# mozack/vdjer

Measured on NVIDIA B200. Metric: graph_build_prune_windows_per_sec, higher is better.
Workload: dtype u8/u64

## Files before the change

vdjer_b200/csrc/kernels.cuh:

```cuda
#pragma once
#include <cstdint>
#include <cuda_runtime.h>

namespace vdjg {

typedef unsigned long long u64;
typedef unsigned int u32;
typedef unsigned short u16;
typedef unsigned char u8;

constexpr u64 EMPTY64 = ~0ull;
constexpr u64 INF64 = ~0ull;
constexpr u32 NIL32 = 0xFFFFFFFFu;
constexpr u32 CNT_CAP = 32765;
constexpr int GATE_Q = 20;
constexpr int HIQ = 30;
constexpr int FLB = 6;
constexpr u32 CNT2_MASK = 0x00FFFFFFu;
constexpr int CNT2_IN = 24;
constexpr u64 LOG_A = 1ull << 62, LOG_B = 1ull << 63;
constexpr int QSUM_SAT = 214;
constexpr int MAX_LOG_RANKS = 11;
constexpr u32 CNT_MULTI = 0x80000000u;
constexpr u32 CNT_SURV = 0x40000000u;
constexpr u32 CNT_MASK = 0x3FFFFFFFu;
constexpr int THREADS = 256;
constexpr int WARPS = THREADS / 32;
constexpr u32 LOG_CHUNK = 64;
constexpr u32 MAX_PROBE = 1u << 14;
constexpr int HIST_BITS = 8;
constexpr int NBUCKET = 1 << HIST_BITS;
constexpr int BHLL_BITS = 7;
constexpr int BHLL = 1 << BHLL_BITS;
constexpr int BATCH = 4;
#ifndef PASS1_MIN_BLOCKS
#define PASS1_MIN_BLOCKS 4
#endif
#ifndef PASS2_MIN_BLOCKS
#define PASS2_MIN_BLOCKS 3
#endif
constexpr int MINI_M = 10;
constexpr int RUN_MAX = 24;
constexpr int SEG_MAX = 32;
constexpr int STAMP_BITS = 40;

struct __align__(32) Slot1 {
    u64 klo, khi;
    u32 count;
    u32 head;
    u32 first_rec;
    u32 first_fp;
};
static_assert(sizeof(Slot1) == 32, "Slot1 must be one sector");

struct __align__(64) Slot2 {
    u64 klo, khi;
    u32 count;
    u32 rank;
    u64 first_any;
    u64 out_first[4];
};
static_assert(sizeof(Slot2) == 64, "Slot2 must be two sectors");


struct Geom {
    int L, k, w, nb, nm;
    int seg;
    int segs;
    u32 tile_rec;
    u64 R;
    u64 n_tiles;
    u64 kmask_lo, kmask_hi;
// ... 176 lines not shown

__device__ __forceinline__ void kmer_succ(u64 lo, u64 hi, u32 c, int k, u64 &slo, u64 &shi) {
    slo = (lo >> 2) | (hi << 62);
    shi = hi >> 2;
    int bit = 2 * (k - 1);
    if (bit < 64) slo |= (u64)c << bit; else shi |= (u64)c << (bit - 64);
}
__device__ __forceinline__ void kmer_pred(u64 lo, u64 hi, u32 c, u64 mlo, u64 mhi, u64 &plo, u64 &phi) {
    phi = ((hi << 2) | (lo >> 62)) & mhi;
    plo = ((lo << 2) | (u64)c) & mlo;
}
__device__ __forceinline__ u32 kmer_last(u64 lo, u64 hi, int k) {
    int bit = 2 * (k - 1);
    return (u32)(bit < 64 ? lo >> bit : hi >> (bit - 64)) & 3u;
}

__device__ __forceinline__ u32 kmer_bucket_of(u64 lo, u64 hi, int span, u32 mmask) {
    u32 minh = ~0u;
    for (int j = 0; j < span; j++) {
        minh = min(minh, mini_hash((u32)lo & mmask));
        lo = (lo >> 2) | (hi << 62);
        hi >>= 2;
    }
    return mini_bucket(minh);
}

template <bool WIDE>
__device__ __forceinline__ void tuple_decode(const Part &pt, u64 w1, u64 w2, u64 &hi, u32 &fl, u32 &fp, u64 &stamp) {
    hi = pt.hb ? (w1 & ((1ull << pt.hb) - 1)) : 0ull;
    fl = (u32)(w1 >> pt.hb) & ((1u << FLB) - 1);
    fp = (u32)(w1 >> (pt.hb + FLB)) & (u32)((1ull << pt.fb) - 1);
    stamp = WIDE ? w2 : (w1 >> (pt.hb + FLB + pt.fb));
}
__device__ __forceinline__ void issue_fence(u32 &a, u32 &b, u32 &c, u32 &d) {
    asm volatile("" : "+r"(a), "+r"(b), "+r"(c), "+r"(d));
}

struct PackArgs {
    const unsigned char *text;
    u64 r0, n;
    u32 fwd_only;
    u64 *bases, *good, *valid, *hiq;
    u8 *qual, *strand;
    u64 *bad;
};
__device__ __forceinline__ u64 spread_bits(u32 a) {
    u64 x = a;
    x = (x | (x << 16)) & 0x0000FFFF0000FFFFull;
    x = (x | (x << 8)) & 0x00FF00FF00FF00FFull;
    x = (x | (x << 4)) & 0x0F0F0F0F0F0F0F0Full;
    x = (x | (x << 2)) & 0x3333333333333333ull;
    x = (x | (x << 1)) & 0x5555555555555555ull;
    return x;
}
__device__ __forceinline__ void pack_record(const PackArgs &a, const Geom &g, const unsigned char *rec, u64 r, bool rev, u32 lane) {
    if (lane == 0) {
        const unsigned sc = rec[0];
        if (sc != '0' && sc != '1') atomicMin(&a.bad[0], r);
        if (sc == '1') a.bad[2] = 1;
        a.strand[r] = (u8)(sc - '0');
    }
    u64 vword = 0, gword = 0, hword = 0;
    for (int j0 = 0; j0 < g.L; j0 += 32) {
        const int j = j0 + (int)lane;
        unsigned code = 4;
        bool okq = false, hiq = false;
        if (j < g.L) {
            const int sj = rev ? g.L - 1 - j : j;
// ... 508 lines not shown
    __device__ __forceinline__ void setup(unsigned char *smem) {
        unsigned char *p = smem + (threadIdx.x >> 5) * bytes();
        lo = reinterpret_cast<u64 *>(p);
        w1 = lo + QC;
        w2 = w1 + QC;
        idx = reinterpret_cast<u32 *>(w1 + (WIDE ? 2 : 1) * QC);
    }
    __host__ __device__ static constexpr size_t bytes() { return (size_t)QC * (WIDE ? 28 : 20); }
    template <class Make>
    __device__ __forceinline__ u32 push_lazy(u32 qn, bool defer, u64 l, u32 i, Make make) {
        const u32 lane = threadIdx.x & 31;
        const u32 ballot = __ballot_sync(0xFFFFFFFFu, defer);
        if (defer) {
            const u32 pos = qn + __popc(ballot & ((1u << lane) - 1));
            u64 a, b;
            make(a, b);
            lo[pos] = l; w1[pos] = a; idx[pos] = i;
            if (WIDE) w2[pos] = b;
        }
        return qn + __popc(ballot);
    }
    __device__ __forceinline__ u32 push(u32 qn, bool defer, u64 l, u64 a, u64 b, u32 i) {
        const u32 lane = threadIdx.x & 31;
        const u32 ballot = __ballot_sync(0xFFFFFFFFu, defer);
        if (defer) {
            const u32 pos = qn + __popc(ballot & ((1u << lane) - 1));
            lo[pos] = l; w1[pos] = a; idx[pos] = i;
            if (WIDE) w2[pos] = b;
        }
        return qn + __popc(ballot);
    }
};

struct RunCursor {
    u64 w0, w1, w2;
    u64 stamp0;
    u32 off, len;
    u32 l;
    u32 j;
    u32 rem;
};
struct RunFeed {
    u64 *rw;
    u32 cnt, incl, total;
    u32 live;
    template <bool GATED_ONLY>
    __device__ __forceinline__ static u32 selected(u64 w2) {
        return GATED_ONLY ? (u32)w2 & 0xFFFFFFu : (1u << run_len(w2)) - 1u;
    }
    template <bool GATED_ONLY>
    __device__ __forceinline__ void load(const u64 *runs, u64 ri, u64 n_runs) {
        const u32 lane = threadIdx.x & 31;
        u64 w0 = 0, w1 = 0, w2 = 0, w3 = 0;
        cnt = 0;
        if (ri < n_runs) {
            ld_run(runs + ri * RUN_WORDS, w0, w1, w2, w3);
            cnt = (u32)__popc(selected<GATED_ONLY>(w2));
        }
        incl = cnt;
        for (int o = 1; o < 32; o <<= 1) { const u32 v = __shfl_up_sync(0xFFFFFFFFu, incl, o); if ((int)lane >= o) incl += v; }
        total = __shfl_sync(0xFFFFFFFFu, incl, 31);
        live = __ballot_sync(0xFFFFFFFFu, cnt != 0);
        __syncwarp();
        u64 *p = rw + lane * RUN_WORDS;
        p[0] = w0; p[1] = w1; p[2] = ri < n_runs ? w2 : 0ull; p[3] = w3;
        __syncwarp();
    }
    template <bool TAB2>
    __device__ __forceinline__ void open(RunCursor &c, const Part &pt) const {
        const u64 *p = rw + c.l * RUN_WORDS;
        c.w0 = p[0]; c.w1 = p[1]; c.w2 = p[2];
        const u64 w3 = p[3];
        c.stamp0 = w3 & ((1ull << STAMP_BITS) - 1);
        const uint4 ut = __ldg(reinterpret_cast<const uint4 *>(pt.ut + (run_bucket(w3) >> pt.ushift)));
        c.off = TAB2 ? ut.z : ut.x;
        c.len = TAB2 ? ut.w : ut.y;
    }
    template <bool GATED_ONLY, bool TAB2>
    __device__ __forceinline__ void seek(u32 t, RunCursor &c, const Part &pt) const {
        u32 l = 0;
#pragma unroll
        for (int s = 16; s; s >>= 1) { const u32 v = __shfl_sync(0xFFFFFFFFu, incl, l + s - 1); if (v <= t) l += s; }
        u32 nth = t - __shfl_sync(0xFFFFFFFFu, incl - cnt, l);
        c.l = l;
        open<TAB2>(c, pt);
        u32 m = selected<GATED_ONLY>(c.w2), j = 0;
        if (GATED_ONLY) {
#pragma unroll
            for (int s = 16; s; s >>= 1) {
                const u32 k = (u32)__popc(m & ((1u << s) - 1u));
                if (nth >= k) { nth -= k; m >>= s; j += s; }
            }
            m >>= 1;
        } else {
            j = nth;
            m >>= j + 1;
        }
        c.j = j; c.rem = m;
    }
    __device__ __forceinline__ u32 fingerprint(u32 l, const Part &pt) const {
        const u64 *p = rw + l * RUN_WORDS;
        return (((u32)(p[3] >> 48) & 0xFFFFu) | (((u32)(p[2] >> 58) & 0x3Fu) << 16)) & (u32)((1ull << pt.fb) - 1);
    }
    template <bool GATED_ONLY, bool TAB2>
    __device__ __forceinline__ void next(RunCursor &c, const Part &pt) const {
        if (c.rem) {
            const u32 s = (u32)__ffs((int)c.rem);
            c.j += s; c.rem >>= s;
            return;
        }
        const u32 ahead = c.l < 31 ? live >> (c.l + 1) : 0u;
        c.l += ahead ? (u32)__ffs((int)ahead) : 0u;
        open<TAB2>(c, pt);
        const u32 m = selected<GATED_ONLY>(c.w2);
        const u32 s = m ? (u32)__ffs((int)m) : 1u;
        c.j = s - 1; c.rem = m >> s;
    }
};
__device__ __forceinline__ void run_kmer(const Geom &g, const RunCursor &c, u64 &lo, u64 &hi, u32 &idx) {
    const u32 sh = 2u * c.j;
    lo = sh ? (c.w0 >> sh) | (c.w1 << (64 - sh)) : c.w0;
    hi = c.w1 >> sh;
    lo &= g.kmask_lo; hi &= g.kmask_hi;
    idx = slot_in(hash_slot(lo, hi), c.off, c.len);
}
__device__ __forceinline__ u32 run_flags(const Geom &g, u64 w0, u64 w1, u64 w2, u32 j) {
    const u32 p = j + (u32)g.k;
    const u32 nb = (u32)((p < 32 ? w0 >> (2 * p) : w1 >> (2 * (p - 32)))) & 3u;
    const bool has_next = j + 1 < run_len(w2) || ((w2 >> 53) & 1ull);
    return (has_next ? 1u | (nb << 1) : 0u) | ((u32)(w2 >> (24 + j)) & 1u) << 3 | ((u32)(w2 >> 54) & 1u) << 4;
}
__device__ __forceinline__ u32 run_flags2(const Geom &g, u64 w0, u64 w1, u64 w2, u32 j) {
    const u32 p = j + (u32)g.k;
    const u32 nb = (u32)((p < 32 ? w0 >> (2 * p) : w1 >> (2 * (p - 32)))) & 3u;
    const bool has_next = j + 1 < run_len(w2) || ((w2 >> 53) & 1ull);
    const u32 prev = j ? 1u | (((u32)(w0 >> (2 * (j - 1))) & 3u) << 1) : (u32)(w2 >> 55) & 7u;
    return (has_next ? 1u | (nb << 1) : 0u) | prev << 3;
}
template <bool WIDE>
__device__ __forceinline__ void pack_tuple(const Part &pt, u64 hi, u32 fl, u32 fp, u64 stamp, u64 &t1, u64 &t2) {
    t1 = hi | ((u64)fl << pt.hb) | ((u64)fp << (pt.hb + FLB));
    if (WIDE) t2 = stamp;
    else { t1 |= stamp << (pt.hb + FLB + pt.fb); t2 = 0; }
}

struct LogCursor { u32 base, used; };

template <bool WIDE>
__device__ __forceinline__ u32 pass1_drain(const Pass1Args &a, const Geom &g, const Part &pt, WarpQueue<WIDE, QCAP1> &q,
                                           u32 qn, LogCursor &lc, bool final) {
    const u32 lane = threadIdx.x & 31, lt = (1u << lane) - 1;
    u32 next = 0;
    bool have = false;
    u64 lo = 0, hi = 0, stamp = 0, rw1 = 0, rw2 = 0;
    u32 idx = 0, probe = 0, fp = 0, fl = 0;
    __syncwarp();
    for (;;) {
        const u32 need = __ballot_sync(0xFFFFFFFFu, !have);
        const u32 avail = qn - next;
        if (avail == 0 && (need == 0xFFFFFFFFu || (!final && 32 - __popc(need) < (int)pt.qdense1))) break;
        if (need && avail) {
            const u32 my = __popc(need & lt);
            if (!have && my < avail) {
                const u32 e = next + my;
                lo = q.lo[e]; rw1 = q.w1[e]; rw2 = WIDE ? q.w2[e] : 0ull;
                tuple_decode<WIDE>(pt, rw1, rw2, hi, fl, fp, stamp);
                idx = q.idx[e];
                probe = 0;
                have = true;
            }
// ... 43 lines not shown
                if (a.nb_ranks && blk != NIL32) a.log[(u64)blk * a.nb_ranks] = entry;
                st_cg_u64(reinterpret_cast<u64 *>(&slot->first_rec), (u64)r | ((u64)fp << 32));
            } else {
                const u32 cw = (u32)q2, cnt = cw & CNT_MASK;
                const u32 first_rec = (u32)q3, first_fp = (u32)(q3 >> 32);
                u32 rank = NIL32;
                if (cnt + 1 < a.nb_ranks) rank = (atomicAdd(&slot->count, 1u) & CNT_MASK) + 1;
                else if (cnt + 1 < CNT_CAP) atomicAdd(&slot->count, 1u);
                if (!(cw & CNT_MULTI) && first_rec != r &&
                    (first_fp != fp || !same_read(a.rd, first_rec, r, g.nb, g.nm)))
                    atomicOr(&slot->count, CNT_MULTI);
                if (rank < a.nb_ranks && blk != NIL32) a.log[(u64)blk * a.nb_ranks + rank] = entry;
            }
            have = false;
        }
    }
    __syncwarp();
    const u32 left = q.push(0, have, lo, rw1, rw2, idx);
    __syncwarp();
    return left;
}

__device__ __forceinline__ void hot_flush(Slot1 *table, u32 *hidx, u32 *hcnt) {
    for (u32 i = threadIdx.x & 31; i < HOTC; i += 32) {
        const u32 c = hcnt[i];
        if (c) {
            u32 *cp = &table[hidx[i]].count;
            if ((*reinterpret_cast<volatile u32 *>(cp) & CNT_MASK) < (1u << 24)) atomicAdd(cp, c);
        }
        hidx[i] = NIL32; hcnt[i] = 0;
    }
}

template <bool WIDE>
__global__ void __launch_bounds__(THREADS, PASS1_MIN_BLOCKS)
k_pass1(Pass1Args a, Geom g, Part pt) {
    extern __shared__ __align__(128) unsigned char smem[];
    WarpQueue<WIDE, QCAP1> q;
    q.setup(smem);
    u32 *hidx = reinterpret_cast<u32 *>(smem + WARPS * WarpQueue<WIDE, QCAP1>::bytes()) + (threadIdx.x >> 5) * 2 * HOTC;
    u32 *hcnt = hidx + HOTC;
    for (u32 i = threadIdx.x & 31; i < HOTC; i += 32) { hidx[i] = NIL32; hcnt[i] = 0; }
    RunFeed feed;
    feed.rw = reinterpret_cast<u64 *>(smem + WARPS * (WarpQueue<WIDE, QCAP1>::bytes() + 2 * HOTC * sizeof(u32))) + (threadIdx.x >> 5) * 32 * RUN_WORDS;
    __syncwarp();
    const u32 lane = threadIdx.x & 31;
    u32 since_flush = 0;
    LogCursor lc; lc.base = 0; lc.used = LOG_CHUNK;
    u32 qn = 0, n_slow = 0;
    const u64 n_chunk = (pt.n_runs + THREADS - 1) / THREADS;
    static_assert(BATCH == 4, "issue_fence takes four operands");
    for (u64 chunk = blockIdx.x; chunk < n_chunk; chunk += gridDim.x) {
        feed.load<true>(a.runs, chunk * THREADS + threadIdx.x, pt.n_runs);
        for (u32 base = 0; base < feed.total; base += 32 * BATCH) {
            u64 lo[BATCH], k0[BATCH], k1[BATCH], m2[BATCH], hi[BATCH];
            u32 idx[BATCH];
            u32 ref[BATCH];
            {
                const u32 t0 = base + lane * BATCH;
                RunCursor cur;
                feed.seek<true, false>(min(t0, feed.total - 1), cur, pt);
#pragma unroll
                for (int u = 0; u < BATCH; u++) {
                    lo[u] = hi[u] = 0; idx[u] = NIL32; ref[u] = 0;
                    if (t0 + u < feed.total) {
                        if (u) feed.next<true, false>(cur, pt);
                        run_kmer(g, cur, lo[u], hi[u], idx[u]);
                        ref[u] = cur.l | (cur.j << 8);
                    }
                }
            }
            issue_fence(idx[0], idx[1], idx[2], idx[3]);
#pragma unroll
            for (int u = 0; u < BATCH; u++) {
                k0[u] = k1[u] = m2[u] = 0;
                if (idx[u] != NIL32) {
                    u64 unused;
                    ld_sector_ca(a.table + idx[u], k0[u], k1[u], m2[u], unused);
                }
            }
#pragma unroll
            for (int u = 0; u < BATCH; u++) {
                const bool valid = idx[u] != NIL32;
                const u32 cw = (u32)m2[u], cnt = cw & CNT_MASK;
                const bool fast = valid && k0[u] == lo[u] && k1[u] == hi[u] && (cw & CNT_MULTI) && cnt + 1 >= a.nb_ranks;
                if (fast && cnt + 1 < CNT_CAP) {
                    bool cached = false;
                    if (cnt >= pt.hot_t) {
                        const u32 e = (idx[u] * 0x9E3779B1u) >> (32 - HOTC_BITS);
                        const u32 old = atomicCAS(&hidx[e], NIL32, idx[u]);
                        if (old == NIL32 || old == idx[u]) { atomicAdd(&hcnt[e], 1u); cached = true; }
                    }
                    if (!cached) atomicAdd(&a.table[idx[u]].count, 1u);
                }
                qn = q.push_lazy(qn, valid && !fast, lo[u], idx[u], [&](u64 &t1, u64 &t2) {
                    const u32 l = ref[u] & 0xFFu, j = ref[u] >> 8;
                    const u64 *p = feed.rw + l * RUN_WORDS;
                    pack_tuple<WIDE>(pt, hi[u], run_flags(g, p[0], p[1], p[2], j), feed.fingerprint(l, pt),
                                     (p[3] & ((1ull << STAMP_BITS) - 1)) + j, t1, t2);
                });
            }
            if (++since_flush >= pt.hot_flush) {
                since_flush = 0;
                __syncwarp();
                hot_flush(a.table, hidx, hcnt);
                __syncwarp();
            }
            if (qn >= pt.qflush1) {
                n_slow += qn; qn = pass1_drain<WIDE>(a, g, pt, q, qn, lc, false); n_slow -= qn;
            }
        }
    }
    __syncwarp();
    hot_flush(a.table, hidx, hcnt);
    n_slow += qn;
    pass1_drain<WIDE>(a, g, pt, q, qn, lc, true);
    if (lane == 0 && n_slow) atomicAdd(&a.ctr->n_slow1, (u64)n_slow);
}

struct PruneArgs {
    Slot1 *table;
    u64 cap;
    const u64 *log;
    u32 nb_ranks;
    Reads rd;
    int mf, T;
    Counters *ctr;
};

__global__ void __launch_bounds__(THREADS)
k_prune(PruneArgs a, Geom g) {
    const u32 lane = threadIdx.x & 31;
    const u64 stride = (u64)gridDim.x * blockDim.x;
    const u64 n_iter = (a.cap + stride - 1) / stride;
    u64 i = (u64)blockIdx.x * blockDim.x + threadIdx.x;
    u32 n_distinct = 0, n_surv = 0;
    for (u64 itn = 0; itn < n_iter; itn++, i += stride) {
        u32 cnt = 0, cw = 0, head = NIL32;
        int lb_first = 0;
        bool pass = false, border = false;
        if (i < a.cap) {
            u64 q0, q1, q2, q3;
            ld_sector(&a.table[i], q0, q1, q2, q3);
            if (!(q0 == EMPTY64 && q1 == EMPTY64)) {
// ... 203 lines not shown
                idx = q.idx[e];
                count_it = idx >> 31;
                idx &= 0x7FFFFFFFu;
                probe = 0;
                have = true;
            }
            next += min((u32)__popc(need), avail);
        }
        if (have) {
            if (++idx == (u32)a.cap) idx = 0;
            Slot2 *slot = a.table + idx;
            u64 q0, q1, q2, q3;
            ld_sector(slot, q0, q1, q2, q3);
            if (q0 == lo && q1 == hi) {
                const u32 c = (fl >> 1) & 3u, coarse = coarse_stamp(stamp, pt.cshift);
                const bool edge = (fl & 1u) && edge_open(q2, c, coarse);
                u64 o = 0;
                if (edge) o = ld_cg_u64(&slot->out_first[c]);
                pass2_update(slot, count_it, q2, q3, o, edge, c, stamp, coarse, fl);
                n_hits++;
                n_hits_u += count_it;
                have = false;
            } else if ((q0 == EMPTY64 && q1 == EMPTY64) || ++probe >= MAX_PROBE) {
                have = false;
            }
        }
    }
    __syncwarp();
    qn = q.push(0, have, lo, rw1, rw2, idx | (count_it ? 0x80000000u : 0u));
    __syncwarp();
    return n_hits;
}

template <bool WIDE>
__global__ void __launch_bounds__(THREADS, PASS2_MIN_BLOCKS)
k_pass2(Pass2Args a, Geom g, Part pt) {
    extern __shared__ __align__(128) unsigned char smem[];
    WarpQueue<WIDE> q;
    q.setup(smem);
    RunFeed feed;
    feed.rw = reinterpret_cast<u64 *>(smem + WARPS * WarpQueue<WIDE>::bytes()) + (threadIdx.x >> 5) * 32 * RUN_WORDS;
    const u32 lane = threadIdx.x & 31;
    const u64 n_chunk = (pt.n_runs + THREADS - 1) / THREADS;
    u32 n_hits = 0, qn = 0, n_slow = 0, n_hits_u = 0;
    for (u64 chunk = blockIdx.x; chunk < n_chunk; chunk += gridDim.x) {
        feed.load<false>(a.runs, chunk * THREADS + threadIdx.x, pt.n_runs);
        for (u32 base = 0; base < feed.total; base += 32 * BATCH) {
            u64 lo[BATCH], hi[BATCH], stamp[BATCH], q0[BATCH], q1[BATCH], q2[BATCH], q3[BATCH], of[BATCH];
            u32 idx[BATCH], fl[BATCH];
            {
                const u32 t0 = base + lane * BATCH;
                RunCursor cur;
                feed.seek<false, true>(min(t0, feed.total - 1), cur, pt);
#pragma unroll
                for (int u = 0; u < BATCH; u++) {
                    lo[u] = hi[u] = stamp[u] = 0; idx[u] = NIL32; fl[u] = 0;
                    if (t0 + u < feed.total) {
                        if (u) feed.next<false, true>(cur, pt);
                        run_kmer(g, cur, lo[u], hi[u], idx[u]);
                        fl[u] = run_flags2(g, cur.w0, cur.w1, cur.w2, cur.j) | ((u32)(cur.w2 >> cur.j) & 1u) << FLB;
                        stamp[u] = cur.stamp0 + cur.j;
                        fl[u] |= coarse_stamp(stamp[u], pt.cshift) << 8;
                    }
                }
            }
            issue_fence(idx[0], idx[1], idx[2], idx[3]);
#pragma unroll
            for (int u = 0; u < BATCH; u++) {
                q0[u] = q1[u] = q2[u] = q3[u] = 0;
                if (idx[u] != NIL32) ld_sector_ca(a.table + idx[u], q0[u], q1[u], q2[u], q3[u]);
            }
            u32 edges = 0;
#pragma unroll
            for (int u = 0; u < BATCH; u++) {
                of[u] = 0;
                if (idx[u] != NIL32 && q0[u] == lo[u] && q1[u] == hi[u] && (fl[u] & 1u) &&
                    edge_open(q2[u], (fl[u] >> 1) & 3u, (fl[u] >> 8) & 0xFFu)) {
                    edges |= 1u << u;
                    of[u] = ld_ca_u64(&a.table[idx[u]].out_first[(fl[u] >> 1) & 3u]);
                }
            }
#pragma unroll
            for (int u = 0; u < BATCH; u++) {
                const bool valid = idx[u] != NIL32;
                const bool ungated = !((fl[u] >> FLB) & 1u);
                const bool hit = valid && q0[u] == lo[u] && q1[u] == hi[u];
                const bool empty = q0[u] == EMPTY64 && q1[u] == EMPTY64;
                if (hit) {
                    pass2_update(a.table + idx[u], ungated, q2[u], q3[u], of[u], (edges >> u) & 1u, (fl[u] >> 1) & 3u, stamp[u],
                                 (fl[u] >> 8) & 0xFFu, fl[u]);
                    n_hits++;
                    n_hits_u += ungated;
                }
                qn = q.push_lazy(qn, valid && !hit && !empty, lo[u], idx[u] | (ungated ? 0x80000000u : 0u), [&](u64 &t1, u64 &t2) {
                    pack_tuple<WIDE>(pt, hi[u], fl[u] & ((1u << FLB) - 1), 0u, stamp[u], t1, t2);
                });
            }
            if (qn >= pt.qflush2) {
                n_slow += qn; n_hits += pass2_drain<WIDE>(a, pt, q, qn, false, n_hits_u); n_slow -= qn;
            }
        }
    }
    n_slow += qn;
    n_hits += pass2_drain<WIDE>(a, pt, q, qn, true, n_hits_u);
    if (lane == 0 && n_slow) atomicAdd(&a.ctr->n_slow2, (u64)n_slow);
    for (int o = 16; o; o >>= 1) { n_hits += __shfl_xor_sync(0xFFFFFFFFu, n_hits, o); n_hits_u += __shfl_xor_sync(0xFFFFFFFFu, n_hits_u, o); }
    if (lane == 0 && n_hits) atomicAdd(&a.ctr->n_hits, (u64)n_hits);
    if (lane == 0 && n_hits_u) atomicAdd(&a.ctr->n_hits_ungated, (u64)n_hits_u);
}

__global__ void __launch_bounds__(THREADS)
k_collect(const Slot2 *t, u64 cap, u64 *keys, u32 *vals, Counters *ctr) {
    u64 i = (u64)blockIdx.x * blockDim.x + threadIdx.x, stride = (u64)gridDim.x * blockDim.x;
    u64 n_iter = (cap + stride - 1) / stride;
    for (u64 itn = 0; itn < n_iter; itn++, i += stride) {
        bool occ = false;
        u64 q0 = 0, q1 = 0, q2 = 0, q3 = 0;
        if (i < cap) {
            ld_sector(&t[i], q0, q1, q2, q3);
            occ = !(q0 == EMPTY64 && q1 == EMPTY64);
        }
        const u64 o = block_append(occ, &ctr->n_nodes);
        if (occ) {
            keys[o] = q3;
            vals[o] = (u32)i;
            if (q3 == INF64) atomicExch(&ctr->internal, 2u);
        }
    }
}

__global__ void k_assign_rank(Slot2 *t, const u32 *vals, u64 n) {
    u64 i = (u64)blockIdx.x * blockDim.x + threadIdx.x;
    if (i < n) t[vals[i]].rank = (u32)i;
}
// ... 343 lines not shown
```

Baseline: 21.86 billion.

## Stream runs per lane with double-buffered batches in pass1 and pass2

Replaces the per-chunk prefix-sum and binary-search seek over runs with per-lane run cursors that refill from a warp-compacted shared-memory chunk, walking k-mers incrementally by shifting. Pass1 and pass2 now ping-pong two step buffers so the table loads for one batch are issued while the previous batch is consumed, and the next run chunk is prefetched into L2. BATCH drops to 2 and the min-blocks launch bounds drop to 2, trading occupancy for more registers and in-flight loads. An A/B profiling script is also added.

```diff
diff --git a/profiles/ab_passes.py b/profiles/ab_passes.py
--- /dev/null
+++ b/profiles/ab_passes.py
@@ -0,0 +1,141 @@
+from __future__ import annotations
+
+import argparse
+import hashlib
+import json
+import os
+import statistics
+import subprocess
+import sys
+import tempfile
+
+import numpy as np
+
+ROOT = os.path.dirname(os.path.dirname(os.path.abspath(__file__)))
+GRAPH_ARRAYS = ["first_pos", "frequency", "out_deg", "in_deg", "out_succ", "in_pred"]
+TIMES = ["ms_device", "ms_pass1", "ms_pass2"]
+COUNTS = ["n_hits", "n_hits_ungated", "n_slow1", "n_slow2", "n_gated", "n_windows"]
+
+
+def worker(args) -> None:
+    sys.path.insert(0, ROOT)
+    from vdjer_b200 import GraphBuilder, synth
+    wl = dict(synth.CONFIGS[args.workload])
+    L, k, mf, mq = wl["read_length"], wl["k"], wl["mf"], wl["mq"]
+    gen = {kk: v for kk, v in wl.items() if kk not in ("k", "mf", "mq")}
+    primary, secondary = synth.generate(seed=12345, pair_offset=0, **gen)
+    with GraphBuilder(L, k, mf, mq, device=0) as gb:
+        gb.stage(primary, secondary)
+        for _ in range(args.warmup):
+            gb.run()
+        per_step = []
+        for _ in range(args.steps):
+            gb.run()
+            per_step.append(gb.fetch_stats())
+        graph = gb.fetch()
+    st = per_step[-1]
+    out = {n: float(np.mean([s[n] for s in per_step])) for n in TIMES}
+    out.update({n: int(st[n]) for n in COUNTS})
+    out["slow_path_fraction_pass1"] = st["n_slow1"] / max(1, st["n_gated"])
+    out["slow_path_fraction_pass2"] = st["n_slow2"] / max(1, st["n_windows"])
+    arrays = {n: np.ascontiguousarray(getattr(graph, n)) for n in GRAPH_ARRAYS}
+    out["n_nodes"] = int(graph.n_nodes)
+    out["sha256"] = {n: hashlib.sha256(a.tobytes()).hexdigest() for n, a in arrays.items()}
+    if args.graph:
+        np.savez(args.graph, **arrays)
+    print("AB_RESULT " + json.dumps(out), flush=True)
+
+
+def run_one(lib: str, args, graph_path: str | None) -> dict:
+    cmd = [sys.executable, os.path.abspath(__file__), "--worker", "--workload", args.workload,
+           "--steps", str(args.steps), "--warmup", str(args.warmup)]
+    if graph_path:
+        cmd += ["--graph", graph_path]
+    env = dict(os.environ, VDJGRAPH_LIB=os.path.abspath(lib))
+    r = subprocess.run(cmd, env=env, capture_output=True, text=True, cwd=ROOT)
+    for line in r.stdout.splitlines():
+        if line.startswith("AB_RESULT "):
+            return json.loads(line[len("AB_RESULT "):])
+    raise SystemExit(f"ab_passes: the process for {lib} failed (exit {r.returncode}):\n{r.stdout[-2000:]}\n{r.stderr[-3000:]}")
+
+
+def gpu_info() -> dict:
+    try:
+        r = subprocess.run(["nvidia-smi", "--query-gpu=name,power.limit,clocks.max.sm", "--format=csv,noheader"],
+                           capture_output=True, text=True, timeout=60)
+        return {"nvidia_smi": r.stdout.strip().splitlines()[:1] or r.stderr.strip()[:200]}
+    except (OSError, subprocess.TimeoutExpired) as e:
+        return {"nvidia_smi": f"unavailable: {e}"}
+
+
+def compare_graphs(path_a: str, path_b: str) -> dict:
+    a, b = np.load(path_a), np.load(path_b)
+    differ = [n for n in GRAPH_ARRAYS if a[n].shape != b[n].shape or not np.array_equal(a[n], b[n])]
+    return {"equal": not differ, "differ": differ, "nodes": int(len(a["first_pos"]))}
+
+
+def summarize(results: list[dict]) -> dict:
+    out = {}
+    for n in TIMES:
+        v = [r[n] for r in results]
+        out[n] = {"median": statistics.median(v), "min": min(v), "max": max(v), "spread": max(v) - min(v)}
+    for n in ["slow_path_fraction_pass1", "slow_path_fraction_pass2", "n_hits", "n_hits_ungated", "n_nodes"]:
+        out[n] = results[-1][n]
+    return out
+
+
+def main():
+    ap = argparse.ArgumentParser(description=__doc__.split("\n")[0])
+    ap.add_argument("libs", nargs="*", help="BASE_LIB NEW_LIB (paths of libvdjgraph.so builds)")
+    ap.add_argument("--workload", default="igh_2x50_5M")
+    ap.add_argument("--reps", type=int, default=5, help="processes per library")
+    ap.add_argument("--steps", type=int, default=10)
+    ap.add_argument("--warmup", type=int, default=3)
+    ap.add_argument("--out", help="also write the summary as JSON to this file")
+    ap.add_argument("--worker", action="store_true", help=argparse.SUPPRESS)
+    ap.add_argument("--graph", help=argparse.SUPPRESS)
+    args = ap.parse_args()
+    if args.worker:
+        worker(args)
+        return
+    if len(args.libs) != 2:
+        ap.error("give two library paths: BASE_LIB NEW_LIB")
+    if args.reps < 1 or args.steps < 1 or args.warmup < 0:
+        ap.error("--reps and --steps must be at least 1, --warmup at least 0")
+    for lib in args.libs:
+        if not os.path.isfile(lib):
+            ap.error(f"no such library: {lib}")
+    sys.path.insert(0, ROOT)
+    from vdjer_b200 import synth
+    if args.workload not in synth.CONFIGS:
+        ap.error(f"unknown workload {args.workload}; one of {sorted(synth.CONFIGS)}")
+
+    names = ["base", "new"]
+    results = {n: [] for n in names}
+    with tempfile.TemporaryDirectory(prefix="ab_passes_") as tmp:
+        graphs = {n: os.path.join(tmp, n + ".npz") for n in names}
+        for rep in range(args.reps):
+            for n, lib in zip(names, args.libs):
+                results[n].append(run_one(lib, args, graphs[n] if rep == 0 else None))
+        graph_cmp = compare_graphs(graphs["base"], graphs["new"])
+    digests_equal = all(r["sha256"] == results["base"][0]["sha256"] for n in names for r in results[n])
+    summary = {"workload": args.workload, "reps": args.reps, "steps": args.steps, "warmup": args.warmup,
+               "gpu": gpu_info(), "libs": dict(zip(names, args.libs)),
+               "base": summarize(results["base"]), "new": summarize(results["new"]),
+               "graphs_equal": graph_cmp["equal"] and digests_equal, "graph_compare": graph_cmp}
+    b, w = summary["base"], summary["new"]
+    for t in TIMES:
+        noise = max(b[t]["spread"], w[t]["spread"])
+        summary[t + "_change"] = {"delta_ms": w[t]["median"] - b[t]["median"], "ratio": w[t]["median"] / b[t]["median"],
+                                  "exceeds_3x_spread": abs(w[t]["median"] - b[t]["median"]) > 3 * noise}
+    summary["hits_equal"] = all(b[n] == w[n] for n in ["n_hits", "n_hits_ungated", "n_nodes"])
+    print(json.dumps(summary, indent=1), flush=True)
+    if args.out:
+        with open(args.out, "w") as f:
+            json.dump(summary, f, indent=1)
+    if not summary["graphs_equal"]:
+        raise SystemExit("ab_passes: the two libraries built different graphs")
+
+
+if __name__ == "__main__":
+    main()
diff --git a/vdjer_b200/csrc/kernels.cuh b/vdjer_b200/csrc/kernels.cuh
--- a/vdjer_b200/csrc/kernels.cuh
+++ b/vdjer_b200/csrc/kernels.cuh
@@ -32,12 +32,15 @@
 constexpr int NBUCKET = 1 << HIST_BITS;
 constexpr int BHLL_BITS = 7;
 constexpr int BHLL = 1 << BHLL_BITS;
-constexpr int BATCH = 4;
+#ifndef PASS_BATCH
+#define PASS_BATCH 2
+#endif
+constexpr int BATCH = PASS_BATCH;
 #ifndef PASS1_MIN_BLOCKS
-#define PASS1_MIN_BLOCKS 4
+#define PASS1_MIN_BLOCKS 2
 #endif
 #ifndef PASS2_MIN_BLOCKS
-#define PASS2_MIN_BLOCKS 3
+#define PASS2_MIN_BLOCKS 2
 #endif
 constexpr int MINI_M = 10;
 constexpr int RUN_MAX = 24;
@@ -280,8 +283,10 @@
     fp = (u32)(w1 >> (pt.hb + FLB)) & (u32)((1ull << pt.fb) - 1);
     stamp = WIDE ? w2 : (w1 >> (pt.hb + FLB + pt.fb));
 }
-__device__ __forceinline__ void issue_fence(u32 &a, u32 &b, u32 &c, u32 &d) {
-    asm volatile("" : "+r"(a), "+r"(b), "+r"(c), "+r"(d));
+template <int N>
+__device__ __forceinline__ void issue_fence(u32 (&a)[N]) {
+#pragma unroll
+    for (int i = 0; i < N; i++) asm volatile("" : "+r"(a[i]));
 }
 
 struct PackArgs {
@@ -856,110 +861,116 @@
     }
 };
 
-struct RunCursor {
-    u64 w0, w1, w2;
-    u64 stamp0;
+template <bool GATED_ONLY>
+struct LaneRun {
+    u64 b0, b1;
+    u64 stamp;
+    u32 sel;
+    u32 aux;
+    u32 left;
+    u32 meta;
     u32 off, len;
-    u32 l;
-    u32 j;
-    u32 rem;
-};
-struct RunFeed {
+    __device__ __forceinline__ void advance() {
+        if (GATED_ONLY) {
+            const u32 rest = sel >> 1, s = (u32)__ffs((int)rest);
+            left = rest ? left - s : 0u;
+            skip(s);
+        } else {
+            meta = (meta & 1u) | (1u | ((u32)b0 & 3u) << 1) << 1;
+            left--;
+            aux >>= 1;
+            stamp++;
+            b0 = (b0 >> 2) | (b1 << 62);
+            b1 >>= 2;
+        }
+    }
+    __device__ __forceinline__ void skip(u32 s) {
+        const u32 sh = 2u * s;
+        sel >>= s; aux >>= s; stamp += s;
+        b0 = (b0 >> sh) | ((b1 << 1) << (63u - sh));
+        b1 >>= sh;
+    }
+    __device__ __forceinline__ u32 next_base(const Geom &g) const {
+        return (u32)(g.k < 32 ? b0 >> (2 * g.k) : b1 >> (2 * g.k - 64)) & 3u;
+    }
+    __device__ __forceinline__ bool has_next() const { return left > 1u || (meta & 1u); }
+};
+template <bool GATED_ONLY, bool TAB2>
+struct RunChunk {
     u64 *rw;
-    u32 cnt, incl, total;
-    u32 live;
-    template <bool GATED_ONLY>
-    __device__ __forceinline__ static u32 selected(u64 w2) {
-        return GATED_ONLY ? (u32)w2 & 0xFFFFFFu : (1u << run_len(w2)) - 1u;
-    }
-    template <bool GATED_ONLY>
-    __device__ __forceinline__ void load(const u64 *runs, u64 ri, u64 n_runs) {
+    u64 wc;
+    u32 nlive, next;
+    __device__ __forceinline__ void setup(u64 *smem_runs) {
+        rw = smem_runs + (threadIdx.x >> 5) * 32 * RUN_WORDS;
+        wc = (u64)blockIdx.x * WARPS + (threadIdx.x >> 5);
+        nlive = next = 0;
+    }
+    __device__ __forceinline__ bool load(const u64 *runs, u64 n_runs) {
         const u32 lane = threadIdx.x & 31;
+        const u64 stride = (u64)gridDim.x * WARPS;
+        if (wc * 32 >= n_runs) return false;
+        const u64 ri = wc * 32 + lane;
         u64 w0 = 0, w1 = 0, w2 = 0, w3 = 0;
-        cnt = 0;
-        if (ri < n_runs) {
-            ld_run(runs + ri * RUN_WORDS, w0, w1, w2, w3);
-            cnt = (u32)__popc(selected<GATED_ONLY>(w2));
-        }
-        incl = cnt;
-        for (int o = 1; o < 32; o <<= 1) { const u32 v = __shfl_up_sync(0xFFFFFFFFu, incl, o); if ((int)lane >= o) incl += v; }
-        total = __shfl_sync(0xFFFFFFFFu, incl, 31);
-        live = __ballot_sync(0xFFFFFFFFu, cnt != 0);
+        if (ri < n_runs) ld_run(runs + ri * RUN_WORDS, w0, w1, w2, w3);
+        if (lane < 8 && (wc + stride) * 32 + 4 * lane < n_runs)
+            asm volatile("prefetch.global.L2 [%0];" :: "l"(runs + ((wc + stride) * 32 + 4 * lane) * RUN_WORDS));
+        const bool live = ri < n_runs && (GATED_ONLY ? ((u32)w2 & 0xFFFFFFu) != 0 : true);
+        const u32 ball = __ballot_sync(0xFFFFFFFFu, live);
         __syncwarp();
-        u64 *p = rw + lane * RUN_WORDS;
-        p[0] = w0; p[1] = w1; p[2] = ri < n_runs ? w2 : 0ull; p[3] = w3;
+        if (live) {
+            ulonglong2 *p = reinterpret_cast<ulonglong2 *>(rw + __popc(ball & ((1u << lane) - 1u)) * RUN_WORDS);
+            p[0] = make_ulonglong2(w0, w1);
+            p[1] = make_ulonglong2(w2, w3);
+        }
         __syncwarp();
-    }
-    template <bool TAB2>
-    __device__ __forceinline__ void open(RunCursor &c, const Part &pt) const {
-        const u64 *p = rw + c.l * RUN_WORDS;
-        c.w0 = p[0]; c.w1 = p[1]; c.w2 = p[2];
-        const u64 w3 = p[3];
-        c.stamp0 = w3 & ((1ull << STAMP_BITS) - 1);
+        nlive = (u32)__popc(ball); next = 0;
+        wc += stride;
+        return true;
+    }
+    __device__ __forceinline__ void open(LaneRun<GATED_ONLY> &r, u32 e, const Part &pt) const {
+        const ulonglong2 *p = reinterpret_cast<const ulonglong2 *>(rw + e * RUN_WORDS);
+        const ulonglong2 a = p[0], b = p[1];
+        const u64 w2 = b.x, w3 = b.y;
+        r.b0 = a.x; r.b1 = a.y;
+        r.stamp = w3 & ((1ull << STAMP_BITS) - 1);
+        r.left = run_len(w2);
         const uint4 ut = __ldg(reinterpret_cast<const uint4 *>(pt.ut + (run_bucket(w3) >> pt.ushift)));
-        c.off = TAB2 ? ut.z : ut.x;
-        c.len = TAB2 ? ut.w : ut.y;
-    }
-    template <bool GATED_ONLY, bool TAB2>
-    __device__ __forceinline__ void seek(u32 t, RunCursor &c, const Part &pt) const {
-        u32 l = 0;
-#pragma unroll
-        for (int s = 16; s; s >>= 1) { const u32 v = __shfl_sync(0xFFFFFFFFu, incl, l + s - 1); if (v <= t) l += s; }
-        u32 nth = t - __shfl_sync(0xFFFFFFFFu, incl - cnt, l);
-        c.l = l;
-        open<TAB2>(c, pt);
-        u32 m = selected<GATED_ONLY>(c.w2), j = 0;
+        r.off = TAB2 ? ut.z : ut.x;
+        r.len = TAB2 ? ut.w : ut.y;
         if (GATED_ONLY) {
-#pragma unroll
-            for (int s = 16; s; s >>= 1) {
-                const u32 k = (u32)__popc(m & ((1u << s) - 1u));
-                if (nth >= k) { nth -= k; m >>= s; j += s; }
-            }
-            m >>= 1;
+            const u32 fp = (((u32)(w3 >> 48) & 0xFFFFu) | (((u32)(w2 >> 58) & 0x3Fu) << 16)) & (u32)((1ull << pt.fb) - 1);
+            r.sel = (u32)w2 & 0xFFFFFFu;
+            r.aux = (u32)(w2 >> 24) & 0xFFFFFFu;
+            r.meta = ((u32)(w2 >> 53) & 3u) | fp << 2;
+            const u32 s = (u32)__ffs((int)r.sel) - 1u;
+            r.left -= s;
+            r.skip(s);
         } else {
-            j = nth;
-            m >>= j + 1;
-        }
-        c.j = j; c.rem = m;
-    }
-    __device__ __forceinline__ u32 fingerprint(u32 l, const Part &pt) const {
-        const u64 *p = rw + l * RUN_WORDS;
-        return (((u32)(p[3] >> 48) & 0xFFFFu) | (((u32)(p[2] >> 58) & 0x3Fu) << 16)) & (u32)((1ull << pt.fb) - 1);
-    }
-    template <bool GATED_ONLY, bool TAB2>
-    __device__ __forceinline__ void next(RunCursor &c, const Part &pt) const {
-        if (c.rem) {
-            const u32 s = (u32)__ffs((int)c.rem);
-            c.j += s; c.rem >>= s;
-            return;
-        }
-        const u32 ahead = c.l < 31 ? live >> (c.l + 1) : 0u;
-        c.l += ahead ? (u32)__ffs((int)ahead) : 0u;
-        open<TAB2>(c, pt);
-        const u32 m = selected<GATED_ONLY>(c.w2);
-        const u32 s = m ? (u32)__ffs((int)m) : 1u;
-        c.j = s - 1; c.rem = m >> s;
-    }
-};
-__device__ __forceinline__ void run_kmer(const Geom &g, const RunCursor &c, u64 &lo, u64 &hi, u32 &idx) {
-    const u32 sh = 2u * c.j;
-    lo = sh ? (c.w0 >> sh) | (c.w1 << (64 - sh)) : c.w0;
-    hi = c.w1 >> sh;
-    lo &= g.kmask_lo; hi &= g.kmask_hi;
-    idx = slot_in(hash_slot(lo, hi), c.off, c.len);
-}
-__device__ __forceinline__ u32 run_flags(const Geom &g, u64 w0, u64 w1, u64 w2, u32 j) {
-    const u32 p = j + (u32)g.k;
-    const u32 nb = (u32)((p < 32 ? w0 >> (2 * p) : w1 >> (2 * (p - 32)))) & 3u;
-    const bool has_next = j + 1 < run_len(w2) || ((w2 >> 53) & 1ull);
-    return (has_next ? 1u | (nb << 1) : 0u) | ((u32)(w2 >> (24 + j)) & 1u) << 3 | ((u32)(w2 >> 54) & 1u) << 4;
-}
-__device__ __forceinline__ u32 run_flags2(const Geom &g, u64 w0, u64 w1, u64 w2, u32 j) {
-    const u32 p = j + (u32)g.k;
-    const u32 nb = (u32)((p < 32 ? w0 >> (2 * p) : w1 >> (2 * (p - 32)))) & 3u;
-    const bool has_next = j + 1 < run_len(w2) || ((w2 >> 53) & 1ull);
-    const u32 prev = j ? 1u | (((u32)(w0 >> (2 * (j - 1))) & 3u) << 1) : (u32)(w2 >> 55) & 7u;
-    return (has_next ? 1u | (nb << 1) : 0u) | prev << 3;
+            r.aux = (u32)w2 & 0xFFFFFFu;
+            r.meta = ((u32)(w2 >> 53) & 1u) | ((u32)(w2 >> 55) & 7u) << 1;
+        }
+    }
+    __device__ __forceinline__ void refill(LaneRun<GATED_ONLY> &r, const u64 *runs, const Part &pt) {
+        const u32 lane = threadIdx.x & 31;
+        for (;;) {
+            const u32 need = __ballot_sync(0xFFFFFFFFu, r.left == 0);
+            if (!need) return;
+            const u32 avail = nlive - next, n = (u32)__popc(need);
+            if (avail) {
+                const u32 my = (u32)__popc(need & ((1u << lane) - 1u));
+                if (r.left == 0 && my < avail) open(r, next + my, pt);
+                next += min(n, avail);
+                if (n <= avail) return;
+            }
+            if (!load(runs, pt.n_runs)) return;
+        }
+    }
+};
+template <bool GATED_ONLY>
+__device__ __forceinline__ void lane_kmer(const Geom &g, const LaneRun<GATED_ONLY> &r, u64 &lo, u64 &hi, u32 &idx) {
+    lo = r.b0 & g.kmask_lo;
+    hi = r.b1 & g.kmask_hi;
+    idx = slot_in(hash_slot(lo, hi), r.off, r.len);
 }
 template <bool WIDE>
 __device__ __forceinline__ void pack_tuple(const Part &pt, u64 hi, u32 fl, u32 fp, u64 stamp, u64 &t1, u64 &t2) {
@@ -1069,6 +1080,11 @@
     }
 }
 
+struct Pass1Step {
+    u64 lo[BATCH], t1[BATCH], t2[BATCH], k0[BATCH], k1[BATCH], m2[BATCH];
+    u32 idx[BATCH];
+};
+
 template <bool WIDE>
 __global__ void __launch_bounds__(THREADS, PASS1_MIN_BLOCKS)
 k_pass1(Pass1Args a, Geom g, Part pt) {
@@ -1078,75 +1094,77 @@
     u32 *hidx = reinterpret_cast<u32 *>(smem + WARPS * WarpQueue<WIDE, QCAP1>::bytes()) + (threadIdx.x >> 5) * 2 * HOTC;
     u32 *hcnt = hidx + HOTC;
     for (u32 i = threadIdx.x & 31; i < HOTC; i += 32) { hidx[i] = NIL32; hcnt[i] = 0; }
-    RunFeed feed;
-    feed.rw = reinterpret_cast<u64 *>(smem + WARPS * (WarpQueue<WIDE, QCAP1>::bytes() + 2 * HOTC * sizeof(u32))) + (threadIdx.x >> 5) * 32 * RUN_WORDS;
+    RunChunk<true, false> feed;
+    feed.setup(reinterpret_cast<u64 *>(smem + WARPS * (WarpQueue<WIDE, QCAP1>::bytes() + 2 * HOTC * sizeof(u32))));
     __syncwarp();
     const u32 lane = threadIdx.x & 31;
+    const u64 hmask = pt.hb ? (1ull << pt.hb) - 1 : 0ull;
     u32 since_flush = 0;
     LogCursor lc; lc.base = 0; lc.used = LOG_CHUNK;
     u32 qn = 0, n_slow = 0;
-    const u64 n_chunk = (pt.n_runs + THREADS - 1) / THREADS;
-    static_assert(BATCH == 4, "issue_fence takes four operands");
-    for (u64 chunk = blockIdx.x; chunk < n_chunk; chunk += gridDim.x) {
-        feed.load<true>(a.runs, chunk * THREADS + threadIdx.x, pt.n_runs);
-        for (u32 base = 0; base < feed.total; base += 32 * BATCH) {
-            u64 lo[BATCH], k0[BATCH], k1[BATCH], m2[BATCH], hi[BATCH];
-            u32 idx[BATCH];
-            u32 ref[BATCH];
-            {
-                const u32 t0 = base + lane * BATCH;
-                RunCursor cur;
-                feed.seek<true, false>(min(t0, feed.total - 1), cur, pt);
+    LaneRun<true> r;
+    r.left = 0;
+    auto expand = [&](Pass1Step &s) -> bool {
+        bool any = false;
 #pragma unroll
-                for (int u = 0; u < BATCH; u++) {
-                    lo[u] = hi[u] = 0; idx[u] = NIL32; ref[u] = 0;
-                    if (t0 + u < feed.total) {
-                        if (u) feed.next<true, false>(cur, pt);
-                        run_kmer(g, cur, lo[u], hi[u], idx[u]);
-                        ref[u] = cur.l | (cur.j << 8);
-                    }
+        for (int u = 0; u < BATCH; u++) {
+            feed.refill(r, a.runs, pt);
+            s.idx[u] = NIL32; s.lo[u] = s.t1[u] = s.t2[u] = 0;
+            if (r.left) {
+                u64 hi;
+                lane_kmer(g, r, s.lo[u], hi, s.idx[u]);
+                const u32 fl = (r.has_next() ? 1u | r.next_base(g) << 1 : 0u) | (r.aux & 1u) << 3 | ((r.meta >> 1) & 1u) << 4;
+                pack_tuple<WIDE>(pt, hi, fl, r.meta >> 2, r.stamp, s.t1[u], s.t2[u]);
+                r.advance();
+                any = true;
+            }
+        }
+        issue_fence(s.idx);
+#pragma unroll
+        for (int u = 0; u < BATCH; u++) {
+            s.k0[u] = s.k1[u] = s.m2[u] = 0;
+            if (s.idx[u] != NIL32) {
+                u64 unused;
+                ld_sector_ca(a.table + s.idx[u], s.k0[u], s.k1[u], s.m2[u], unused);
+            }
+        }
+        return __any_sync(0xFFFFFFFFu, any);
+    };
+    auto consume = [&](const Pass1Step &s) {
+#pragma unroll
+        for (int u = 0; u < BATCH; u++) {
+            const bool valid = s.idx[u] != NIL32;
+            const u32 cw = (u32)s.m2[u], cnt = cw & CNT_MASK;
+            const bool fast = valid && s.k0[u] == s.lo[u] && s.k1[u] == (s.t1[u] & hmask) && (cw & CNT_MULTI) && cnt + 1 >= a.nb_ranks;
+            if (fast && cnt + 1 < CNT_CAP) {
+                bool cached = false;
+                if (cnt >= pt.hot_t) {
+                    const u32 e = (s.idx[u] * 0x9E3779B1u) >> (32 - HOTC_BITS);
+                    const u32 old = atomicCAS(&hidx[e], NIL32, s.idx[u]);
+                    if (old == NIL32 || old == s.idx[u]) { atomicAdd(&hcnt[e], 1u); cached = true; }
                 }
-            }
-            issue_fence(idx[0], idx[1], idx[2], idx[3]);
-#pragma unroll
-            for (int u = 0; u < BATCH; u++) {
-                k0[u] = k1[u] = m2[u] = 0;
-                if (idx[u] != NIL32) {
-                    u64 unused;
-                    ld_sector_ca(a.table + idx[u], k0[u], k1[u], m2[u], unused);
-                }
-            }
-#pragma unroll
-            for (int u = 0; u < BATCH; u++) {
-                const bool valid = idx[u] != NIL32;
-                const u32 cw = (u32)m2[u], cnt = cw & CNT_MASK;
-                const bool fast = valid && k0[u] == lo[u] && k1[u] == hi[u] && (cw & CNT_MULTI) && cnt + 1 >= a.nb_ranks;
-                if (fast && cnt + 1 < CNT_CAP) {
-                    bool cached = false;
-                    if (cnt >= pt.hot_t) {
-                        const u32 e = (idx[u] * 0x9E3779B1u) >> (32 - HOTC_BITS);
-                        const u32 old = atomicCAS(&hidx[e], NIL32, idx[u]);
-                        if (old == NIL32 || old == idx[u]) { atomicAdd(&hcnt[e], 1u); cached = true; }
-                    }
-                    if (!cached) atomicAdd(&a.table[idx[u]].count, 1u);
-                }
-                qn = q.push_lazy(qn, valid && !fast, lo[u], idx[u], [&](u64 &t1, u64 &t2) {
-                    const u32 l = ref[u] & 0xFFu, j = ref[u] >> 8;
-                    const u64 *p = feed.rw + l * RUN_WORDS;
-                    pack_tuple<WIDE>(pt, hi[u], run_flags(g, p[0], p[1], p[2], j), feed.fingerprint(l, pt),
-                                     (p[3] & ((1ull << STAMP_BITS) - 1)) + j, t1, t2);
-                });
-            }
-            if (++since_flush >= pt.hot_flush) {
-                since_flush = 0;
-                __syncwarp();
-                hot_flush(a.table, hidx, hcnt);
-                __syncwarp();
-            }
-            if (qn >= pt.qflush1) {
-                n_slow += qn; qn = pass1_drain<WIDE>(a, g, pt, q, qn, lc, false); n_slow -= qn;
-            }
-        }
+                if (!cached) atomicAdd(&a.table[s.idx[u]].count, 1u);
+            }
+            qn = q.push(qn, valid && !fast, s.lo[u], s.t1[u], s.t2[u], s.idx[u]);
+        }
+        if (++since_flush >= pt.hot_flush) {
+            since_flush = 0;
+            __syncwarp();
+            hot_flush(a.table, hidx, hcnt);
+            __syncwarp();
+        }
+        if (qn >= pt.qflush1) {
+            n_slow += qn; qn = pass1_drain<WIDE>(a, g, pt, q, qn, lc, false); n_slow -= qn;
+        }
+    };
+    Pass1Step x, y;
+    bool more = expand(x);
+    while (more) {
+        const bool more_y = expand(y);
+        consume(x);
+        if (!more_y) break;
+        more = expand(x);
+        consume(y);
     }
     __syncwarp();
     hot_flush(a.table, hidx, hcnt);
@@ -1416,74 +1434,90 @@
     return n_hits;
 }
 
+struct Pass2Step {
+    u64 lo[BATCH], hi[BATCH], stamp[BATCH], q0[BATCH], q1[BATCH], q2[BATCH], q3[BATCH], of[BATCH];
+    u32 idx[BATCH], fl[BATCH];
+    u32 edges;
+};
+
 template <bool WIDE>
 __global__ void __launch_bounds__(THREADS, PASS2_MIN_BLOCKS)
 k_pass2(Pass2Args a, Geom g, Part pt) {
     extern __shared__ __align__(128) unsigned char smem[];
     WarpQueue<WIDE> q;
     q.setup(smem);
-    RunFeed feed;
-    feed.rw = reinterpret_cast<u64 *>(smem + WARPS * WarpQueue<WIDE>::bytes()) + (threadIdx.x >> 5) * 32 * RUN_WORDS;
+    RunChunk<false, true> feed;
+    feed.setup(reinterpret_cast<u64 *>(smem + WARPS * WarpQueue<WIDE>::bytes()));
     const u32 lane = threadIdx.x & 31;
-    const u64 n_chunk = (pt.n_runs + THREADS - 1) / THREADS;
     u32 n_hits = 0, qn = 0, n_slow = 0, n_hits_u = 0;
-    for (u64 chunk = blockIdx.x; chunk < n_chunk; chunk += gridDim.x) {
-        feed.load<false>(a.runs, chunk * THREADS + threadIdx.x, pt.n_runs);
-        for (u32 base = 0; base < feed.total; base += 32 * BATCH) {
-            u64 lo[BATCH], hi[BATCH], stamp[BATCH], q0[BATCH], q1[BATCH], q2[BATCH], q3[BATCH], of[BATCH];
-            u32 idx[BATCH], fl[BATCH];
-            {
-                const u32 t0 = base + lane * BATCH;
-                RunCursor cur;
-                feed.seek<false, true>(min(t0, feed.total - 1), cur, pt);
+    LaneRun<false> r;
+    r.left = 0;
+    auto expand = [&](Pass2Step &s) -> bool {
+        bool any = false;
 #pragma unroll
-                for (int u = 0; u < BATCH; u++) {
-                    lo[u] = hi[u] = stamp[u] = 0; idx[u] = NIL32; fl[u] = 0;
-                    if (t0 + u < feed.total) {
-                        if (u) feed.next<false, true>(cur, pt);
-                        run_kmer(g, cur, lo[u], hi[u], idx[u]);
-                        fl[u] = run_flags2(g, cur.w0, cur.w1, cur.w2, cur.j) | ((u32)(cur.w2 >> cur.j) & 1u) << FLB;
-                        stamp[u] = cur.stamp0 + cur.j;
-                        fl[u] |= coarse_stamp(stamp[u], pt.cshift) << 8;
-                    }
-                }
-            }
-            issue_fence(idx[0], idx[1], idx[2], idx[3]);
+        for (int u = 0; u < BATCH; u++) {
+            feed.refill(r, a.runs, pt);
+            s.lo[u] = s.hi[u] = s.stamp[u] = 0; s.idx[u] = NIL32; s.fl[u] = 0;
+            if (r.left) {
+                lane_kmer(g, r, s.lo[u], s.hi[u], s.idx[u]);
+                s.stamp[u] = r.stamp;
+                s.fl[u] = (r.has_next() ? 1u | r.next_base(g) << 1 : 0u) | ((r.meta >> 1) & 7u) << 3 | (r.aux & 1u) << FLB |
+                          coarse_stamp(r.stamp, pt.cshift) << 8;
+                r.advance();
+                any = true;
+            }
+        }
+        issue_fence(s.idx);
 #pragma unroll
-            for (int u = 0; u < BATCH; u++) {
-                q0[u] = q1[u] = q2[u] = q3[u] = 0;
-                if (idx[u] != NIL32) ld_sector_ca(a.table + idx[u], q0[u], q1[u], q2[u], q3[u]);
-            }
-            u32 edges = 0;
+        for (int u = 0; u < BATCH; u++) {
+            s.q0[u] = s.q1[u] = s.q2[u] = s.q3[u] = 0;
+            if (s.idx[u] != NIL32) ld_sector_ca(a.table + s.idx[u], s.q0[u], s.q1[u], s.q2[u], s.q3[u]);
+        }
+        return __any_sync(0xFFFFFFFFu, any);
+    };
+    auto load_edges = [&](Pass2Step &s) {
+        s.edges = 0;
 #pragma unroll
-            for (int u = 0; u < BATCH; u++) {
-                of[u] = 0;
-                if (idx[u] != NIL32 && q0[u] == lo[u] && q1[u] == hi[u] && (fl[u] & 1u) &&
-                    edge_open(q2[u], (fl[u] >> 1) & 3u, (fl[u] >> 8) & 0xFFu)) {
-                    edges |= 1u << u;
-                    of[u] = ld_ca_u64(&a.table[idx[u]].out_first[(fl[u] >> 1) & 3u]);
-                }
-            }
+        for (int u = 0; u < BATCH; u++) {
+            s.of[u] = 0;
+            if (s.idx[u] != NIL32 && s.q0[u] == s.lo[u] && s.q1[u] == s.hi[u] && (s.fl[u] & 1u) &&
+                edge_open(s.q2[u], (s.fl[u] >> 1) & 3u, (s.fl[u] >> 8) & 0xFFu)) {
+                s.edges |= 1u << u;
+                s.of[u] = ld_ca_u64(&a.table[s.idx[u]].out_first[(s.fl[u] >> 1) & 3u]);
+            }
+        }
+    };
+    auto consume = [&](const Pass2Step &s) {
 #pragma unroll
-            for (int u = 0; u < BATCH; u++) {
-                const bool valid = idx[u] != NIL32;
-                const bool ungated = !((fl[u] >> FLB) & 1u);
-                const bool hit = valid && q0[u] == lo[u] && q1[u] == hi[u];
-                const bool empty = q0[u] == EMPTY64 && q1[u] == EMPTY64;
-                if (hit) {
-                    pass2_update(a.table + idx[u], ungated, q2[u], q3[u], of[u], (edges >> u) & 1u, (fl[u] >> 1) & 3u, stamp[u],
-                                 (fl[u] >> 8) & 0xFFu, fl[u]);
-                    n_hits++;
-                    n_hits_u += ungated;
-                }
-                qn = q.push_lazy(qn, valid && !hit && !empty, lo[u], idx[u] | (ungated ? 0x80000000u : 0u), [&](u64 &t1, u64 &t2) {
-                    pack_tuple<WIDE>(pt, hi[u], fl[u] & ((1u << FLB) - 1), 0u, stamp[u], t1, t2);
-                });
-            }
-            if (qn >= pt.qflush2) {
-                n_slow += qn; n_hits += pass2_drain<WIDE>(a, pt, q, qn, false, n_hits_u); n_slow -= qn;
-            }
-        }
+        for (int u = 0; u < BATCH; u++) {
+            const bool valid = s.idx[u] != NIL32;
+            const bool ungated = !((s.fl[u] >> FLB) & 1u);
+            const bool hit = valid && s.q0[u] == s.lo[u] && s.q1[u] == s.hi[u];
+            const bool empty = s.q0[u] == EMPTY64 && s.q1[u] == EMPTY64;
+            if (hit) {
+                pass2_update(a.table + s.idx[u], ungated, s.q2[u], s.q3[u], s.of[u], (s.edges >> u) & 1u, (s.fl[u] >> 1) & 3u,
+                             s.stamp[u], (s.fl[u] >> 8) & 0xFFu, s.fl[u]);
+                n_hits++;
+                n_hits_u += ungated;
+            }
+            qn = q.push_lazy(qn, valid && !hit && !empty, s.lo[u], s.idx[u] | (ungated ? 0x80000000u : 0u), [&](u64 &t1, u64 &t2) {
+                pack_tuple<WIDE>(pt, s.hi[u], s.fl[u] & ((1u << FLB) - 1), 0u, s.stamp[u], t1, t2);
+            });
+        }
+        if (qn >= pt.qflush2) {
+            n_slow += qn; n_hits += pass2_drain<WIDE>(a, pt, q, qn, false, n_hits_u); n_slow -= qn;
+        }
+    };
+    Pass2Step x, y;
+    bool more = expand(x);
+    while (more) {
+        load_edges(x);
+        const bool more_y = expand(y);
+        consume(x);
+        if (!more_y) break;
+        load_edges(y);
+        more = expand(x);
+        consume(y);
     }
     n_slow += qn;
     n_hits += pass2_drain<WIDE>(a, pt, q, qn, true, n_hits_u);
```

Measured after the change: 17.56 billion (median of 6 runs). 0.803x the previous value.
